# yezhen17/3DIoUMatch

Hardware: AMD Instinct MI355X
Metric: scenes/sec train-step (ScanNet 40k pts, 256 proposals) (higher is better)
Workload: dtype f32

## Files before the change

### 3dioumatch_amd/_lib.py

```python
import ctypes
import os

_HERE = os.path.dirname(os.path.abspath(__file__))
LIB_PATH = os.path.join(_HERE, "lib3dioumatch_hip%s.so" % os.environ.get("PN2_LIB_SUFFIX", ""))

_c_int, _c_float, _vp, _sz = ctypes.c_int, ctypes.c_float, ctypes.c_void_p, ctypes.c_size_t


class MlpOperand(ctypes.Structure):
    _fields_ = [("mode", _c_int), ("x", _vp), ("dz", _vp), ("scale", _vp), ("shift", _vp), ("mean", _vp),
                ("invstd", _vp), ("coef", _vp), ("argmax", _vp), ("ns", _c_int), ("groups", _c_int),
                ("lin_w", _vp)]


_op = ctypes.POINTER(MlpOperand)

_SIGNATURES = {
    "pn2_furthest_point_sampling": [_c_int, _c_int, _c_int, _vp, _vp, _vp, _vp],
    "pn2_furthest_point_sampling_ws": [_c_int, _c_int, _c_int, _vp, _vp, _vp, _sz, _vp],
    "pn2_fps_workspace_bytes": [_c_int, _c_int, _c_int],
    "pn2_gather_points": [_c_int, _c_int, _c_int, _c_int, _vp, _vp, _vp, _vp],
    "pn2_gather_points_grad": [_c_int, _c_int, _c_int, _c_int, _vp, _vp, _vp, _vp],
    "pn2_ball_query": [_c_int, _c_int, _c_int, _c_float, _c_int, _vp, _vp, _vp, _vp, _sz, _vp],
    "pn2_ball_query_workspace_bytes": [_c_int, _c_int, _c_int, _c_int],
# ... 40 lines not shown
    "mlp_bn_workspace_floats": [_c_int, _c_int, _c_int],
    "mlp_bn_train_stats": [_c_int, _c_int, _c_int, _vp, _vp, _vp, _c_float, _c_float, _vp, _vp, _vp,
                           _vp, _vp, _vp, _vp, _vp, _vp],
    "mlp_bn_eval_coeff": [_c_int, _vp, _vp, _c_float, _vp, _vp, _vp, _vp, _vp, _vp, _vp],
    "mlp_bn_relu_apply": [_c_int, _c_int, _c_int, _vp, _vp, _vp, _vp, _vp],
    "mlp_bn_relu_pool": [_c_int, _c_int, _c_int, _c_int, _vp, _vp, _vp, _vp, _vp, _vp, _vp],
    "mlp_bn_relu_backward": [_c_int, _c_int, _c_int, _c_int, _vp, _vp, _vp, _vp, _vp, _vp, _vp, _vp,
                             _vp, _vp, _vp, _vp, _vp, _vp],
    "mlp_bn_relu_pool_backward": [_c_int, _c_int, _c_int, _c_int, _c_int, _vp, _vp, _vp, _vp, _vp,
                                  _vp, _vp, _vp, _vp, _vp, _vp, _vp, _vp, _vp, _vp, _vp],
    "mlp_bn_relu_backward_stats": [_c_int, _c_int, _c_int, _c_int, _vp, _vp, _vp, _vp, _vp, _vp,
                                   _vp, _vp, _vp, _vp, _vp, _vp, _vp],
    "mlp_gemm_forward": [_c_int] * 4 + [_vp, _vp, _op, _vp, _vp, _vp],
    "mlp_gemm_forward_small": [_c_int] * 4 + [_vp, _c_int, _vp, _op, _vp, _vp, _vp],
    "mlp_gemm_forward_stats_parts": [_c_int, _c_int, _c_int, _c_int, _vp],
    "mlp_bn_finalize_pairs": [_c_int, _c_int, _c_int, _vp, _vp, _vp, _c_float, _c_float, _vp, _vp,
                              _vp, _vp, _vp, _vp, _vp, _vp],
    "mlp_bn_finalize_pairs_scratch_bytes": [_c_int],
    "mlp_gemm_dgrad": [_c_int] * 4 + [_vp, _op, _vp, _vp],
    "mlp_gemm_wgrad": [_c_int] * 4 + [_op, _op, _vp, _vp, _vp],
    "mlp_gemm_wgrad_workspace_floats": [_c_int, _c_int, _c_int, _c_int],
    "mlp_gemm_forward_stats_pool_supported": [_c_int, _c_int, _c_int, _c_int, _c_int],
    "mlp_gemm_forward_stats_pool": [_c_int] * 4 + [_vp, _op, _vp, _vp, _c_int, _vp, _vp, _vp],
    "mlp_pool_gram_supported": [_c_int] * 5,
    "mlp_pool_gram_parts": [_c_int] * 4,
    "mlp_pool_gram_workspace_floats": [_c_int] * 5,
    "mlp_pool_gram_backward": [_c_int] * 4 + [_vp, _op, _op] + [_vp] * 6,
    "mlp_eval_lin4_supported": [_c_int] * 6,
    "mlp_eval_lin4_pool": [_c_int, _c_int, _c_int, _vp, _vp, _vp, _vp, _vp, _vp, _vp, _vp],
    "mlp_eval_stored_supported": [_c_int] * 6,
    "mlp_eval_stored_tiles_per_wave": [_c_int] * 4,
    "mlp_eval_stored_image_bytes": [_c_int],
    "mlp_eval_stored_prepare": [_c_int, _vp, _vp, _vp, _vp],
    "mlp_eval_stored_pool": [_c_int, _c_int, _c_int, _c_int, _vp, _vp, _vp, _vp, _vp, _vp, _vp, _vp, _vp, _vp],
    "mlp_chain_lin4_parts": [_c_int, _c_int, _c_int, _c_int, _vp],
    "mlp_chain_lin4_image_bytes": [],
    "mlp_chain_lin4_prepare": [_vp, _vp, _vp, _vp, _vp, _vp, _vp],
    "mlp_chain_lin4_stats": [_c_int, _c_int, _c_int, _vp, _vp, _vp, _vp],
    "mlp_chain_lin4_forward": [_c_int, _c_int, _c_int, _vp, _vp, _vp, _vp, _vp, _vp, _vp, _vp, _vp, _vp],
    "mlp_chain_finalize": [_c_int, _c_int, _c_int, _vp, _vp, _vp, _c_float, _c_float, _vp, _vp, _vp, _vp, _vp,
                           _vp, _vp],
    "mlp_bn_pool_from_extrema": [_c_int, _c_int, _c_int, _vp, _vp, _vp, _vp, _vp, _vp, _vp],
    "mlp_wgrad_first4_workspace_bytes": [_c_int, _c_int],
    "mlp_wgrad_first4": [_c_int, _c_int, _vp, _vp, _vp, _vp, _vp, _vp, _vp, _vp, _vp, _vp, _vp, _vp],
    "mlp_wgrad_first4_from_gated": [_c_int] + [_vp] * 9,
    "mlp_first4_moments_doubles": [],
# ... 124 lines not shown
```

### 3dioumatch_amd/csrc/mlp_gemm.hip

```cpp
#include "common.h"
#include "mlp_operand.h"
#include <mutex>
#include <stdlib.h>

namespace {

constexpr int KC = 16;

template <int TM, int TN, int WM, int WN, int MODE, bool A_TRANS>
__global__ void __launch_bounds__(256)
gemm_nn_kernel(int m_total, int k_total, int r, const float *__restrict__ a, int lda, OperandB opb,
               float *__restrict__ c, size_t b_stride_in, size_t b_stride_out) {
  constexpr int MB = TM / WM / 32, NB = TN / WN / 32;
  constexpr int LDA = TM + 4;
  __shared__ float As[KC * LDA];
  __shared__ __attribute__((aligned(16))) float Bs[KC * TN];
  const int tid = threadIdx.x, lane = tid & 63, wave = tid >> 6;
  const int wm = wave / WN, wn = wave % WN;
  const int r0 = blockIdx.x * TN, m0 = blockIdx.y * TM, b = blockIdx.z;
  OperandB op = opb;
  const size_t in_off = (size_t)b * b_stride_in;

  f32x16 acc[MB][NB];
#pragma unroll
// ... 1249 lines not shown
    return launch_nn<OP_BNRELU>(b, m, k, r, w, ldw, op, y, in_stride, out_stride, stream, nullptr, ai);
  }
  const dim3 grid(pn2_ceil_div(r, 64), pn2_ceil_div(m, 64), b);
#define BIAS_FORM(MODE)                                                                                  \
  do {                                                                                                   \
    if (img)                                                                                             \
      hipLaunchKernelGGL((gemm_nn_small_bias_kernel<MODE, true>), grid, dim3(256), 0, stream, m, k, r, w, \
                         ldw, op, y, in_stride, out_stride, ai, bias);                                   \
    else                                                                                                 \
      hipLaunchKernelGGL((gemm_nn_small_bias_kernel<MODE, false>), grid, dim3(256), 0, stream, m, k, r,  \
                         w, ldw, op, y, in_stride, out_stride, ai, bias);                                \
  } while (0)
  if (x->mode == OP_DIRECT) BIAS_FORM(OP_DIRECT);
  else BIAS_FORM(OP_BNRELU);
#undef BIAS_FORM
  return pn2_launch_status();
}

MLP_API int mlp_gemm_forward_stats_pool_supported(int b, int m, int k, int r, int ns) {
  if (mlp_gemm_forward_stats_parts(b, m, k, r, nullptr) == 0) return 0;
  return (m == 128 || m == 256) && (ns == 16 || ns == 32 || ns == 64) && r % ns == 0 && k % 4 == 0;
}

MLP_API int mlp_gemm_forward_stats_pool(int b, int m, int k, int r, const float *w, const MlpOperand *x,
                                        float *y, float *pairs, int ns, const float *gamma, float *ext,
                                        void *stream_) {
  if (!mlp_gemm_forward_stats_pool_supported(b, m, k, r, ns)) return (int)hipErrorInvalidValue;
  OperandB op;
  const int rc = operand_from_abi(x, op_bit(OP_BNRELU), r, &op);
  if (rc) return rc;
  if (!pairs || !ext || !gamma || (reinterpret_cast<size_t>(w) & 15) != 0) return (int)hipErrorInvalidValue;
  hipStream_t stream = (hipStream_t)stream_;
  if (mlp_pool_fwd256_supported(b, m, k, r, ns, w, *x) && (reinterpret_cast<size_t>(y) & 15) == 0)
    return mlp_pool_fwd256_launch(b, r, ns, w, *x, gamma, y, pairs, ext, stream);
  const size_t in_stride = (size_t)k * r, out_stride = (size_t)m * r;
  const size_t plane = (size_t)b * m * (r / ns);
  const unsigned a_bytes = (unsigned)(4 * (size_t)m * k);
#define POOLED(TM, TN, WM, WN, NS)                                                                 \
  hipLaunchKernelGGL((gemm_nn2_kernel<TM, TN, WM, WN, OP_BNRELU, false, true, true, NS>),          \
                     dim3(r / TN, 1, b), dim3(256), 0, stream, m, k, r, w, k, a_bytes, op, y,     \
                     in_stride, out_stride, pairs, m, ext, plane, gamma)
  if (m == 256 && ns == 16) POOLED(256, 64, 4, 1, 16);
  else if (m == 256 && ns == 32) POOLED(256, 64, 4, 1, 32);
  else if (m == 256) POOLED(256, 64, 4, 1, 64);
  else if (ns == 16) POOLED(128, 128, 2, 2, 16);
  else if (ns == 32) POOLED(128, 128, 2, 2, 32);
  else POOLED(128, 128, 2, 2, 64);
#undef POOLED
  return pn2_launch_status();
}

MLP_API int mlp_gemm_dgrad(int b, int m, int k, int r, const float *w, const MlpOperand *dy,
                           float *dx, void *stream_) {
  if (b <= 0 || m <= 0 || k <= 0 || r <= 0) return 0;
  OperandB op;
  const int rc = operand_from_abi(dy, op_bit(OP_DIRECT) | op_bit(OP_DY) | op_bit(OP_POOLDY), r, &op);
  if (rc) return rc;
  const size_t in_stride = (size_t)m * r, out_stride = (size_t)k * r;
  hipStream_t stream = (hipStream_t)stream_;
  if (dy->mode == OP_DIRECT)
    return launch_nn<OP_DIRECT, true>(b, k, m, r, w, k, op, dx, in_stride, out_stride, stream);
  if (dy->mode == OP_DY)
    return launch_nn<OP_DY, true>(b, k, m, r, w, k, op, dx, in_stride, out_stride, stream);
  return launch_nn<OP_POOLDY, true>(b, k, m, r, w, k, op, dx, in_stride, out_stride, stream);
}

static bool wgrad_direct_ok(int b, int m, int k, int r, int pmode, int qmode);
static int wgrad_direct_r_per_slice(int b, int m, int k, int r);

MLP_API int mlp_gemm_backward_small_supported(int b, int m, int k, int r, int pmode, int qmode) {
  return b > 0 && m > 0 && k > 0 && (long long)b * r <= small_gemm_cols() &&
         wgrad_direct_ok(b, m, k, r, pmode, qmode);
// ... 147 lines not shown
```

### 3dioumatch_amd/csrc/mlp_operand.h

```cpp
#pragma once
#include "common.h"
#include "mlp_frag.h"
#include "../../include/mlp_hip.h"

namespace {

enum OperandMode { OP_DIRECT = 0, OP_BNRELU = 1, OP_DY = 2, OP_POOLDY = 3, OP_LIN4 = 4 };

struct OperandB {
  const float *x;
  const float *dz;
  const float *scale;
  const float *shift;
  const float *mean;
  const float *invstd;
  const float *coef;
  const int *argmax;
  int ns;
  int groups;
  const float *lin_w;
};

constexpr bool is_dy(int mode) { return mode == OP_DY || mode == OP_POOLDY; }

// ... 83 lines not shown
        if (MODE == OP_DY) {
          const float4 d = *reinterpret_cast<const float4 *>(op.dz + off + i);
          dz[i] = d.x; dz[i + 1] = d.y; dz[i + 2] = d.z; dz[i + 3] = d.w;
        }
      }
    }
  } else {
#pragma unroll
    for (int i = 0; i < N; ++i) {
      if (gr + i < limit) {
        x[i] = op.x[off + i];
        if (MODE == OP_DY) dz[i] = op.dz[off + i];
      }
    }
  }
}

}

int mlp_reduce_partials(int count, int parts, const float *part, float *out, hipStream_t stream);
int mlp_reduce_weight_partials(int count, int parts, const float *part, float *out, hipStream_t stream);
int mlp_pool_fwd256_supported(int b, int m, int k, int r, int ns, const float *w, const MlpOperand &x);
int mlp_pool_fwd256_launch(int b, int r, int ns, const float *w, const MlpOperand &x, const float *gamma,
                           float *y, float *pairs, float *ext, hipStream_t stream);
bool mlp_pool_gram256_supported(int b, int r, int ns);
int mlp_pool_gram256_parts(int b, int r);
size_t mlp_pool_gram256_workspace_floats(int b, int r, int ns);
int mlp_pool_gram256_launch(int b, int r, const float *w, const MlpOperand &dy, const MlpOperand &x,
                            const float *ymax, float *dq, float *dw, float *stats_part, float *workspace,
                            hipStream_t stream);
```

### 3dioumatch_amd/csrc/mlp_pool_fwd256.hip

```cpp
#include "common.h"
#include "mlp_operand.h"
#include <stdlib.h>
#include <type_traits>

namespace {

constexpr int kFM = 256, kFK = 128, kFTN = 32;
constexpr int kFRP = kFTN * 2;
constexpr int kFIMG = kFK * kFRP;
constexpr int kFBUF = 3 * kFIMG;
constexpr int kFTP = 32 * 144;

struct PoolFwdArgs {
  int r, chunks_per_cloud, total_tiles, groups;
  const float *w;
  const float *x;
  const float *sc, *sh;
  const float *gamma;
  float *pairs;
  float *ext;
  size_t ext_plane;
  float *y;
};

typedef float f_f32x2 __attribute__((ext_vector_type(2)));
typedef float f_f32x4 __attribute__((ext_vector_type(4)));

template <int NS, bool STORE>
__global__ void __launch_bounds__(512) pool_fwd256_kernel(const PoolFwdArgs a) {
  constexpr int K = kFK, TN = kFTN, RP = kFRP, IMG = kFIMG, BUF = kFBUF;
  constexpr int G = TN / NS;
  constexpr int QG = 16 / G;
  static_assert(NS == 16 || NS == 32, "nsample");
  extern __shared__ __attribute__((aligned(16))) char lds[];

  const int tid = threadIdx.x, lane = tid & 63;
  const int wave = __builtin_amdgcn_readfirstlane(tid >> 6);
  const int l31 = lane & 31, lhi = lane >> 5;
  const int seg_row = tid >> 3, seg_c = (tid & 7) * 4;
  const int ch = 32 * wave + l31;

  Split3 wsp[K / 16];
  {
    const float *wr = a.w + (size_t)ch * K + 8 * lhi;
#pragma unroll
    for (int s = 0; s < K / 16; ++s)
      wsp[s] = split3(*reinterpret_cast<const float4 *>(wr + 16 * s),
                      *reinterpret_cast<const float4 *>(wr + 16 * s + 4));
  }
  const bool neg = a.gamma[ch] < 0.f;
  const float sg = neg ? -1.f : 1.f;
  const f_f32x2 sgn = {sg, sg};
  const RowCoef rc0 = {a.sc[seg_row], a.sh[seg_row], 0.f, 0.f, 0.f};
  const RowCoef rc1 = {a.sc[seg_row + 64], a.sh[seg_row + 64], 0.f, 0.f, 0.f};

  const int blocks = a.total_tiles / 2;
  const int per = (blocks + (int)gridDim.x - 1) / (int)gridDim.x;
  const int k_lo = (int)blockIdx.x * per;
  const int k_hi = k_lo + per < blocks ? k_lo + per : blocks;
  const int c_lo = 4 * k_lo, c_hi = 4 * k_hi;
  if (c_lo >= c_hi) return;

  float4 qx0, qx1, qf0, qf1;
  auto fetch = [&](int c) {
    const int b = c / a.chunks_per_cloud;
    const int col0 = (c - b * a.chunks_per_cloud) * TN;
    const float *src = a.x + ((size_t)b * K + seg_row) * a.r + col0 + seg_c;
    qf0 = *reinterpret_cast<const float4 *>(src);
    qf1 = *reinterpret_cast<const float4 *>(src + (size_t)64 * a.r);
  };
  auto stage_slice = [&](char *base, int row, const float4 &x, const RowCoef &rc) {
    const float xv[4] = {x.x, x.y, x.z, x.w};
    float h[4], m[4], l[4];
#pragma unroll
    for (int e = 0; e < 4; ++e) split_terms(transform<OP_BNRELU>(xv[e], 0.f, rc), h[e], m[e], l[e]);
    store_terms4<RP>(base, IMG, row, seg_c, h, m, l);
  };
  auto stage = [&](char *base) {
    stage_slice(base, seg_row, qx0, rc0);
    stage_slice(base, seg_row + 64, qx1, rc1);
  };
  auto clampc = [&](int c) { return c < c_hi ? c : c_hi - 1; };

  const int tr_off = (8 * lhi + ((lane & 15) >> 2)) * RP + (16 * ((lane >> 4) & 1) + 4 * (lane & 3)) * 2;
  bf16x4 pf[2][3][2];
  auto frag = [&](const char *Q, int s, bf16x4 (&dst)[3][2]) {
#pragma unroll
    for (int t = 0; t < 3; ++t) {
      const char *p0 = Q + (size_t)t * IMG + (size_t)(16 * s) * RP + tr_off;
      dst[t][0] = lds_read_tr(p0);
      dst[t][1] = lds_read_tr(p0 + 4 * RP);
    }
  };
  auto operand = [&](const bf16x4 (&src)[3][2]) {
    Split3 sb;
    sb.hi = __builtin_shufflevector(src[0][0], src[0][1], 0, 1, 2, 3, 4, 5, 6, 7);
    sb.mid = __builtin_shufflevector(src[1][0], src[1][1], 0, 1, 2, 3, 4, 5, 6, 7);
    sb.lo = __builtin_shufflevector(src[2][0], src[2][1], 0, 1, 2, 3, 4, 5, 6, 7);
    return sb;
  };

  fetch(c_lo);
  qx0 = qf0; qx1 = qf1;
  stage(lds);
  fetch(clampc(c_lo + 1));
  qx0 = qf0; qx1 = qf1;
  fetch(clampc(c_lo + 2));
  __syncthreads();
  frag(lds, 0, pf[0]);

  float tsh = 0.f;
  f_f32x2 t1 = {0.f, 0.f}, t2 = {0.f, 0.f};
  unsigned held[4] = {0u, 0u, 0u, 0u};
  int cur = 0;

  float sv[4], shh[4], sm[4], sl[4];
  f_f32x2 pv[8];
  float best[G], mh = 0.f, qh = 0.f, mo = 0.f, qo = 0.f;
  float ob[G];
  int at[G], oa[G];
  char *Qn = lds;
  int ce = 0;
  bool real = false;
  f_f32x4 yrow[2];
  auto store_rows = [&](int k0) {
    if (real) {
      const int b = ce / a.chunks_per_cloud;
      float *dst = a.y + ((size_t)b * kFM + 32 * wave + (lane >> 3)) * a.r + (ce - b * a.chunks_per_cloud) * TN + 4 * (lane & 7);
#pragma unroll
      for (int k2 = 0; k2 < 2; ++k2)
        __builtin_nontemporal_store(yrow[k2], reinterpret_cast<f_f32x4 *>(dst + (size_t)(8 * (k0 + k2)) * a.r));
    }
  };
  auto piece = [&](auto nt) {
    constexpr int n = decltype(nt)::value;
    if constexpr (n == 0 || n == 4) {
      const float4 &x = n == 0 ? qx0 : qx1;
      const RowCoef &rc = n == 0 ? rc0 : rc1;
      const float xv[4] = {x.x, x.y, x.z, x.w};
#pragma unroll
      for (int e = 0; e < 4; ++e) sv[e] = transform<OP_BNRELU>(xv[e], 0.f, rc);
    } else if constexpr (n == 1 || n == 5) {
#pragma unroll
      for (int e = 0; e < 4; ++e) split_top(sv[e], shh[e], sv[e]);
    } else if constexpr (n == 2 || n == 6) {
#pragma unroll
      for (int e = 0; e < 4; ++e) split_top(sv[e], sm[e], sl[e]);
    } else if constexpr (n == 3 || n == 7) {
      store_terms4<RP>(Qn, IMG, seg_row + (n == 7 ? 64 : 0), seg_c, shh, sm, sl);
    } else if constexpr (n == 8) {
      qx0 = qf0; qx1 = qf1;
      fetch(clampc(ce + 4));
    } else if constexpr (n == 9 || n == 10 || n == 11) {
      if (n == 9 && (ce & 1) == 0) { tsh = pv[0].x; t1 = f_f32x2{0.f, 0.f}; t2 = t1; }
      if constexpr (STORE) {
        char *tp = lds + 3 * BUF + wave * kFTP;
        if constexpr (n == 9) {
#pragma unroll
          for (int j = 0; j < 4; ++j)
            *reinterpret_cast<f_f32x4 *>(tp + l31 * 144 + 32 * j + 16 * lhi) =
                f_f32x4{pv[2 * j].x, pv[2 * j].y, pv[2 * j + 1].x, pv[2 * j + 1].y};
        } else if constexpr (n == 10) {
#pragma unroll
          for (int k2 = 0; k2 < 2; ++k2) yrow[k2] = *reinterpret_cast<const f_f32x4 *>(tp + (8 * k2 + (lane >> 3)) * 144 + (lane & 7) * 16);
        } else {
          store_rows(0);
#pragma unroll
          for (int k2 = 0; k2 < 2; ++k2) yrow[k2] = *reinterpret_cast<const f_f32x4 *>(tp + (8 * (k2 + 2) + (lane >> 3)) * 144 + (lane & 7) * 16);
        }
      }
      const f_f32x2 sh2 = {tsh, tsh};
#pragma unroll
      for (int j = 3 * (n - 9); j < (n == 11 ? 8 : 3 * (n - 8)); ++j) {
        const f_f32x2 d = pv[j] - sh2;
        t1 += d;
// ... 34 lines not shown
#pragma unroll
      for (int gq = 0; gq < G; ++gq) {
        float bb = best[gq];
        int aa = at[gq];
        if (ob[gq] > bb || (ob[gq] == bb && oa[gq] < aa)) { bb = ob[gq]; aa = oa[gq]; }
        if (aa == 64) aa = 0;
        const float out = bb * sg;
        held[0] = held[1]; held[1] = held[2]; held[2] = held[3];
        held[3] = lhi == 0 ? __builtin_bit_cast(unsigned, out) : (unsigned)aa;
      }
    } else if constexpr (n == 19) {
      if (ce & 1) {
        const float s1 = t1.x + t1.y, s2 = t2.x + t2.y;
        mh = tsh + s1 * (1.0f / 32.0f);
        qh = fmaxf(s2 - s1 * s1 * (1.0f / 32.0f), 0.f);
        mo = __shfl_xor(mh, 32, kWave);
        qo = __shfl_xor(qh, 32, kWave);
      }
    } else if constexpr (n == 20) {
      if ((ce & 1) && real && lhi == 0) {
        const float dlt = mo - mh;
        const float mean = 0.5f * (mh + mo);
        const float m2w = (qh + qo) + 16.0f * dlt * dlt;
        *reinterpret_cast<float2 *>(a.pairs + ((size_t)(ce >> 1) * kFM + ch) * 2) = make_float2(mean, m2w);
      }
    } else if constexpr (n == 21) {
      if ((ce & (4 / G - 1)) == 4 / G - 1 && real) {
        const int b = ce / a.chunks_per_cloud;
        const int g_last = ((ce - b * a.chunks_per_cloud) * TN) / NS + G - 1;
        const size_t o = ((size_t)b * kFM + ch) * a.groups + g_last - 3 + (lhi ? a.ext_plane : 0);
        *reinterpret_cast<uint4 *>(reinterpret_cast<unsigned *>(a.ext) + o) = make_uint4(held[0], held[1], held[2], held[3]);
      }
    }
  };
#define PF_PIECE(N) do { piece(std::integral_constant<int, (N)>{}); __builtin_amdgcn_sched_barrier(0); } while (0)

#pragma unroll
  for (int j = 0; j < 8; ++j) pv[j] = f_f32x2{0.f, 0.f};
  for (int c = c_lo; c < c_hi; ++c) {
    const int nxt = cur == 2 ? 0 : cur + 1;
    const char *Qc = lds + (size_t)cur * BUF;
    Qn = lds + (size_t)nxt * BUF;
    ce = c - 1;
    real = c > c_lo;
    f32x16 acc, acc1;
#pragma unroll
    for (int q = 0; q < 16; ++q) { acc[q] = 0.f; acc1[q] = 0.f; }
#pragma unroll
    for (int s = 0; s < K / 16; ++s) {
      const int ring = s & 1;
      if (s + 1 < K / 16) frag(Qc, s + 1, pf[ring ^ 1]);
      else frag(Qn, 0, pf[ring ^ 1]);
      __builtin_amdgcn_sched_barrier(0);
      const Split3 x = operand(pf[ring]);
      const Split3 &w = wsp[s];
#define PF_MM(AT, BT)                                                                                \
  acc = __builtin_amdgcn_mfma_f32_32x32x16_bf16(x.AT, w.BT, acc, 0, 0, 0);
#define PF_MM1(AT, BT)                                                                               \
  acc1 = __builtin_amdgcn_mfma_f32_32x32x16_bf16(x.AT, w.BT, acc1, 0, 0, 0);
#define PF_CASE(N) case N: PF_PIECE(N); break
      PF_MM(lo, hi) PF_MM1(hi, lo)
      switch (3 * s) {
        PF_CASE(0); PF_CASE(3); PF_CASE(6); PF_CASE(9); PF_CASE(12); PF_CASE(15); PF_CASE(18); PF_CASE(21);
      }
      PF_MM(mid, mid) PF_MM1(mid, hi)
      switch (3 * s + 1) {
        PF_CASE(1); PF_CASE(4); PF_CASE(7); PF_CASE(10); PF_CASE(13); PF_CASE(16); PF_CASE(19);
      }
      PF_MM(hi, mid) PF_MM1(hi, hi)
      switch (3 * s + 2) {
        PF_CASE(2); PF_CASE(5); PF_CASE(8); PF_CASE(11); PF_CASE(14); PF_CASE(20);
      }
#undef PF_CASE
#undef PF_MM
#undef PF_MM1
      if (s == 3) __syncthreads();
    }
    cur = nxt;
#pragma unroll
    for (int j = 0; j < 8; ++j) pv[j] = f_f32x2{acc[2 * j], acc[2 * j + 1]} + f_f32x2{acc1[2 * j], acc1[2 * j + 1]};
  }
  ce = c_hi - 1;
  real = true;
  PF_PIECE(9); PF_PIECE(10); PF_PIECE(11); PF_PIECE(12); PF_PIECE(13); PF_PIECE(14); PF_PIECE(15);
  PF_PIECE(16); PF_PIECE(18); PF_PIECE(19); PF_PIECE(20); PF_PIECE(21);
#undef PF_PIECE
}

}

int mlp_pool_fwd256_supported(int b, int m, int k, int r, int ns, const float *w, const MlpOperand &x) {
  const char *env = getenv("MLP_POOL_FWD256");
  const bool off = env && atoi(env) == 0;
  if (off || b <= 0 || m != kFM || k != kFK || r <= 0 || r % 256 != 0) return 0;
  if ((ns != 16 && ns != 32) || r % ns != 0) return 0;
  return ((reinterpret_cast<size_t>(w) | reinterpret_cast<size_t>(x.x)) & 15) == 0 ? 1 : 0;
}

int mlp_pool_fwd256_launch(int b, int r, int ns, const float *w, const MlpOperand &x, const float *gamma,
                           float *y, float *pairs, float *ext, hipStream_t stream) {
  if (!w || !x.x || !x.scale || !x.shift || !gamma || !pairs || !ext || (ns != 16 && ns != 32) || b <= 0 || r <= 0 ||
      r % 256 != 0)
    return (int)hipErrorInvalidValue;
  PoolFwdArgs a = {};
  a.r = r; a.chunks_per_cloud = r / kFTN; a.total_tiles = b * (r / 64); a.groups = r / ns;
  a.w = w; a.x = x.x; a.sc = x.scale; a.sh = x.shift; a.gamma = gamma; a.pairs = pairs; a.ext = ext; a.y = y;
  a.ext_plane = (size_t)b * kFM * (size_t)(r / ns);
  int grid = pn2_cu_count();
  if (grid > a.total_tiles / 2) grid = a.total_tiles / 2;
  const size_t kLds = 3 * (size_t)kFBUF + (y != nullptr ? 8 * (size_t)kFTP : 0);
  constexpr size_t kLdsMax = 3 * (size_t)kFBUF + 8 * (size_t)kFTP;
  for (const void *kern : {reinterpret_cast<const void *>(pool_fwd256_kernel<16, false>),
                           reinterpret_cast<const void *>(pool_fwd256_kernel<32, false>),
                           reinterpret_cast<const void *>(pool_fwd256_kernel<16, true>),
                           reinterpret_cast<const void *>(pool_fwd256_kernel<32, true>)})
    pn2_allow_dynamic_lds(kern, kLdsMax);
  if (y != nullptr) {
    if (ns == 16) hipLaunchKernelGGL((pool_fwd256_kernel<16, true>), dim3(grid), dim3(512), kLds, stream, a);
    else hipLaunchKernelGGL((pool_fwd256_kernel<32, true>), dim3(grid), dim3(512), kLds, stream, a);
  } else {
    if (ns == 16) hipLaunchKernelGGL((pool_fwd256_kernel<16, false>), dim3(grid), dim3(512), kLds, stream, a);
    else hipLaunchKernelGGL((pool_fwd256_kernel<32, false>), dim3(grid), dim3(512), kLds, stream, a);
  }
  return pn2_launch_status();
}
```

### 3dioumatch_amd/dropin/pointnet2/_mlp_ext.py

```python
import contextlib
import ctypes
import os

import torch

from pointnet2._ext import _L, _lib, _stream

SMALL_BWD_DY_COLS = 4096


def _f32c(t, name):
    if t.dtype != torch.float32 or not t.is_contiguous() or not t.is_cuda:
        raise RuntimeError("%s must be a contiguous float32 GPU tensor" % name)


def _ws(y, b, c, r):
    n = int(_lib.mlp_bn_workspace_floats(b, c, r))
    return torch.empty(max(n, 1), dtype=torch.float32, device=y.device)


def new_tickets(channels, device):
    return torch.zeros(max(int(channels), 1), dtype=torch.int32, device=device)


def tickets_of(module, channels, device):
    t = module.__dict__.get("_pn2_tickets")
    if t is None or t.device != device or t.numel() < channels:
        t = new_tickets(channels, device)
        module.__dict__["_pn2_tickets"] = t
    return t


def _tk(tickets, c, ref):
    if tickets is None:
        return new_tickets(c, ref.device)
    if tickets.dtype != torch.int32 or tickets.device != ref.device or tickets.numel() < c or \
            not tickets.is_contiguous():
        raise RuntimeError("tickets must be a contiguous int32 tensor of >= %d zeros on %s" % (c, ref.device))
    return tickets


def bn_coefficients(y, gamma, beta, running_mean, running_var, momentum, eps, training, tickets=None):
    _f32c(y, "y")
    b, c = y.shape[0], y.shape[1]
    r = y.numel() // (b * c)
    out = torch.empty((4, c), dtype=torch.float32, device=y.device)
    mean, invstd, scale, shift = out[0], out[1], out[2], out[3]
    with torch.cuda.device(y.device):
        if training:
            ws = _ws(y, b, c, r)
            rm = running_mean.data_ptr() if running_mean is not None else None
            rv = running_var.data_ptr() if running_var is not None else None
            _L.check(_lib.mlp_bn_train_stats(b, c, r, y.data_ptr(), gamma.data_ptr(),
                                             beta.data_ptr(), float(eps), float(momentum), rm, rv,
                                             mean.data_ptr(), invstd.data_ptr(), scale.data_ptr(),
                                             shift.data_ptr(), ws.data_ptr(),
                                             _tk(tickets, c, y).data_ptr(), _stream(y)),
                     "mlp_bn_train_stats")
        else:
            _L.check(_lib.mlp_bn_eval_coeff(c, gamma.data_ptr(), beta.data_ptr(), float(eps),
                                            running_mean.data_ptr(), running_var.data_ptr(),
                                            mean.data_ptr(), invstd.data_ptr(), scale.data_ptr(),
# ... 220 lines not shown
    y = torch.empty((b, m) + tuple(x.shape[2:]), dtype=torch.float32, device=x.device)
    image = _image_of(w, b, r)
    op = _input_operand(x, coeff)
    with torch.cuda.device(x.device):
        _L.check(_lib.mlp_gemm_forward(b, m, k, r, w.data_ptr(), image[0] if image else None,
                                       ctypes.byref(op), y.data_ptr(), None, _stream(x)),
                 "mlp_gemm_forward")
    return y


def _finalize_pairs(c, parts, n_part, pairs, gamma, beta, running_mean, running_var, momentum, eps):
    out = torch.empty((4, c), dtype=torch.float32, device=pairs.device)
    scratch = torch.empty(int(_lib.mlp_bn_finalize_pairs_scratch_bytes(c)), dtype=torch.uint8,
                          device=pairs.device)
    _L.check(_lib.mlp_bn_finalize_pairs(c, parts, n_part, pairs.data_ptr(), gamma.data_ptr(),
                                        beta.data_ptr(), float(eps), float(momentum),
                                        _ptr(running_mean), _ptr(running_var), out[0].data_ptr(),
                                        out[1].data_ptr(), out[2].data_ptr(), out[3].data_ptr(),
                                        scratch.data_ptr(), _stream(pairs)), "mlp_bn_finalize_pairs")
    return out[0], out[1], out[2], out[3]


def gemm_forward_bn(w, x, coeff, gamma, beta, running_mean, running_var, momentum, eps, pool=False,
                    tickets=None, store=True):
    _f32c(x, "x"); _f32c(w, "w")
    b, k = x.shape[0], x.shape[1]
    r = x.numel() // (b * k)
    m = w.shape[0]
    cols = ctypes.c_int(0)
    parts = int(_lib.mlp_gemm_forward_stats_parts(b, m, k, r, ctypes.byref(cols)))
    if parts <= 0:
        y = gemm_forward(w, x, coeff)
        return (y,) + tuple(bn_coefficients(y, gamma, beta, running_mean, running_var, momentum,
                                            eps, True, tickets)) + ((None,) if pool else ())
    ns = x.shape[3] if (pool and x.dim() == 4) else 0
    pooled = bool(ns) and coeff is not None and w.data_ptr() % 16 == 0 and \
        bool(_lib.mlp_gemm_forward_stats_pool_supported(b, m, k, r, ns))
    ext = torch.empty((2, b, m, r // ns), dtype=torch.float32, device=x.device) if pooled else None
    if not store and not pooled:
        raise RuntimeError("gemm_forward_bn(store=False): the pooled epilogue does not cover this layer")
    y = torch.empty((b, m) + tuple(x.shape[2:]), dtype=torch.float32, device=x.device) if store else None
    pairs = torch.empty((parts, m, 2), dtype=torch.float32, device=x.device)
    op = _input_operand(x, coeff)
    with torch.cuda.device(x.device):
        if pooled:
            _L.check(_lib.mlp_gemm_forward_stats_pool(b, m, k, r, w.data_ptr(), ctypes.byref(op), _ptr(y),
                                                      pairs.data_ptr(), ns, gamma.data_ptr(),
                                                      ext.data_ptr(), _stream(x)),
                     "mlp_gemm_forward_stats_pool")
        else:
            _L.check(_lib.mlp_gemm_forward(b, m, k, r, w.data_ptr(), None, ctypes.byref(op),
                                           y.data_ptr(), pairs.data_ptr(), _stream(x)),
                     "mlp_gemm_forward(pairs)")
        bn = _finalize_pairs(m, parts, cols.value, pairs, gamma, beta, running_mean, running_var,
                             momentum, eps)
    return (y,) + bn + ((ext,) if pool else ())


def forward_pool_supported(w, x, coeff):
    shape = x if isinstance(x, tuple) else tuple(x.shape)
    if len(shape) != 4 or coeff is None or w.data_ptr() % 16 != 0:
        return False
    b, k, m, ns = shape
    return bool(_lib.mlp_gemm_forward_stats_pool_supported(b, w.shape[0], k, m * ns, ns))


def pool_from_extrema(ext, scale, shift):
    _, b, c, m = ext.shape
# ... 489 lines not shown
```

### 3dioumatch_amd/dropin/pointnet2/pytorch_utils.py

```python
import contextlib
import os

import torch
import torch.nn as nn
from torch.autograd import Function


class _BNBase(nn.Sequential):

    def __init__(self, in_size, batch_norm=None, name=""):
        super().__init__()
        layer = batch_norm(in_size)
        nn.init.constant_(layer.weight, 1.0)
        nn.init.constant_(layer.bias, 0)
        self.add_module(name + "bn", layer)


class BatchNorm1d(_BNBase):
    def __init__(self, in_size, *, name=""):
        super().__init__(in_size, batch_norm=nn.BatchNorm1d, name=name)


class BatchNorm2d(_BNBase):
    def __init__(self, in_size, name=""):
# ... 142 lines not shown
        raise RuntimeError("the pre-gather form needs src_ext (B, 3+C, n+m) and two layers or more")
    first = "plain"
    if isinstance(pre, Pregathered):
        first = "pregathered"
    elif isinstance(pre, Interpolated):
        first = "interpolated"
    elif training and n >= 3 and x.dim() == 4 and not input_grad and K.lin4_supported(ws[0], ws[1], x):
        chained = pool and n == 3 and K.chain_lin4_supported(ws[0], ws[1], ws[2], x, x.shape[3])
        first = "chained" if chained else "virtual"
    if not pool:
        return first, "apply"
    b, m, ns = pre.extent if pre is not None else (x.shape[0], x.shape[2], x.shape[3])
    y_in = (b, ws[-1].shape[1], m, ns)
    if first == "chained":
        return first, "gram" if K.pool_gram_supported(ws[2], y_in, ns) else "extrema"
    if not (training and n >= 2 and K.forward_pool_supported(ws[-1], y_in, True)):
        return first, "bn_relu_pool"
    return first, "gram" if K.pool_gram_supported(ws[-1], y_in, ns) else "extrema"


class _FusedMLPChain(Function):

    @staticmethod
    def forward(ctx, x, pool, training, momenta, epss, pre, tickets, *params):
        from pointnet2 import _mlp_ext as K
        n = len(params) // 5
        x = x.contiguous()
        ws = [w.reshape(w.shape[0], -1) for w in params[0::5]]
        bns = [tuple(params[5 * i + 1:5 * i + 5]) + (momenta[i], epss[i]) for i in range(n)]
        first, last = chain_forms(ws, x, pre, pool, training, ctx.needs_input_grad[0])
        store = any(ctx.needs_input_grad)
        ys, coefs = [], []
        moments, ext = None, None
        if first in ("virtual", "chained"):
            moments = K.first4_moments(x)
            ys.append(None)
            coefs.append(K.first4_bn(moments, x.numel() // 4, ws[0], *bns[0]))
        if first == "chained":
            y1, c1, y2, c2, ext = K.chain_lin4_forward(x, ws[0], coefs[0][2:], (ws[1],) + bns[1],
                                                       (ws[2],) + bns[2], store=store, store_last=last != "gram")
            ys += [y1, y2]
            coefs += [c1, c2]
        elif first == "virtual":
            y, *c = K.gemm_forward_bn_lin4(ws[1], x, ws[0], coefs[0][2:], *bns[1])
            ys.append(y)
            coefs.append(tuple(c))
        elif first == "pregathered" and training:
            y, *c = pre.forward(ws[0], x, bns[0])
            ys.append(y)
            coefs.append(tuple(c))
        elif pre is not None:
            ys.append(pre.forward(ws[0], x))
            coefs.append(K.bn_coefficients(ys[0], *bns[0], training, tickets))
        for i in range(len(ys), n):
            cur, coeff = (x, None) if i == 0 else (ys[i - 1], coefs[i - 1][2:])
            if i == n - 1 and last in ("extrema", "gram"):
                y, *c, ext = K.gemm_forward_bn(ws[i], cur, coeff, *bns[i], pool=True, tickets=tickets,
                                               store=store and last == "extrema")
            elif training:
                y, *c = K.gemm_forward_bn(ws[i], cur, coeff, *bns[i], tickets=tickets)
            else:
                y = K.gemm_forward(ws[i], cur, coeff)
                c = K.bn_coefficients(y, *bns[i], False, tickets)
            ys.append(y)
            coefs.append(tuple(c))
        scale, shift = coefs[-1][2:]
        argmax = ymax = None
        if last == "apply":
            out = K.bn_relu_apply(ys[-1], scale, shift)
        elif last == "bn_relu_pool":
            out, argmax, ymax = K.bn_relu_pool(ys[-1], scale, shift)
        else:
            out, argmax, ymax = K.pool_from_extrema(ext, scale, shift)
        ctx.save_for_backward(x, moments, argmax, ymax, *ys, *[t for c in coefs for t in c], *params)
        ctx.n_layers, ctx.training, ctx.tickets, ctx.pre = n, training, tickets, pre
        ctx.first, ctx.last = first, last
        return out

    @staticmethod
    def backward(ctx, dout):
        from pointnet2 import _mlp_ext as K
# ... 39 lines not shown
            if i == 0 and first == "pregathered":
                dw, dz = ctx.pre.backward(ws[0], x, grad["fly"], need_dx)
                grads[0] = dw.view_as(params[0])
                break
            lin_w = ws[0] if (i == 1 and virtual) else None
            src = x if (i == 0 or lin_w is not None) else ys[i - 1]
            src_coeff = None if i == 0 else coefs[i - 1][2:]
            src_stats = None if i == 0 else coefs[i - 1][:2] + (params[5 * i - 4], training)
            fused = None if "dy" in grad else K.gemm_backward_fused(
                ws[i], src, src_coeff, xstats=src_stats, need_dx=i > 0 or need_dx, lin_w=lin_w, **grad)
            if fused is not None:
                dsrc, dw, below = fused
            elif lin_w is not None:
                raise RuntimeError("the virtual first layer needs the fused backward kernel of the second")
            elif i == 0 and not need_dx:
                dsrc, below = None, None
                dw = K.wgrad_first4(ws[0], x, grad["fly"]) if "fly" in grad else None
                if dw is None:
                    dw = K.gemm_wgrad(ws[0].shape[0], ws[0].shape[1], x, None, **grad)
            else:
                (dw, dsrc), below = K.both(ws[i], src, src_coeff, **grad), None
            grads[5 * i] = dw.view_as(params[5 * i])
            dz = dsrc
        return (dz if need_dx else None, None, None, None, None, None, None, *grads)


_deferred_counters = None
_deferred_axpy = None
zero_grads_as_none = False


@contextlib.contextmanager
def deferred_bn_counters():
    global _deferred_counters, _deferred_axpy
    previous, _deferred_counters = _deferred_counters, []
    previous_axpy, _deferred_axpy = _deferred_axpy, []
    try:
        yield
    finally:
        pending, _deferred_counters = _deferred_counters, previous
        axpy, _deferred_axpy = _deferred_axpy, previous_axpy
        if pending:
            torch._foreach_add_(pending, 1)
        by_alpha = {}
        for t, other, alpha in axpy:
            by_alpha.setdefault(float(alpha), ([], []))
            by_alpha[float(alpha)][0].append(t)
# ... 45 lines not shown
            return False
        conv, bn_wrap, act = kids["conv"], kids["bn"], kids["activation"]
        bns = list(bn_wrap.children())
        return (isinstance(conv, nn.Conv2d) and conv.kernel_size == (1, 1) and conv.bias is None
                and conv.stride == (1, 1) and conv.padding == (0, 0) and len(bns) == 1
                and isinstance(bns[0], nn.BatchNorm2d) and bns[0].affine
                and bns[0].track_running_stats and bns[0].momentum is not None
                and isinstance(act, nn.ReLU))

    def _use_fused(self, x):
        return (x.is_cuda and x.dtype == torch.float32 and x.dim() == 4 and len(self) > 0
                and all(self._fusable(layer) for layer in self))

    def _run(self, x, pool, pre=None):
        from pointnet2 import _mlp_ext as K
        if _eval_plans is not None and pool:
            plan = _eval_plans.get(id(self))
            if plan is not None and plan.mlp is self:
                out = plan.run(x, pre)
                if out is not None:
                    return out
        layers = list(self)
        tickets = K.tickets_of(self, max(layer.conv.out_channels for layer in layers), x.device)
        bns = [next(layer.bn.children()) for layer in layers]
        training = bns[0].training
        if all(bn.training == training for bn in bns):
            params = []
            for layer, bn in zip(layers, bns):
                if training:
                    bump_batches_tracked(bn.num_batches_tracked)
                params += [layer.conv.weight, bn.weight, bn.bias, bn.running_mean,
                           bn.running_var]
            return _FusedMLPChain.apply(x, pool, training, [bn.momentum for bn in bns],
                                        [bn.eps for bn in bns], pre, tickets, *params)
        for i, layer in enumerate(layers):
            bn = next(layer.bn.children())
            y = layer.conv(x)
            training = bn.training
            if training:
                bump_batches_tracked(bn.num_batches_tracked)
            op = _BNReLUMaxPool if (pool and i == len(layers) - 1) else _BNReLU
            x = op.apply(y, bn.weight, bn.bias, bn.running_mean, bn.running_var, bn.momentum,
                         bn.eps, training, tickets)
        return x

    def forward(self, x):
        if self._use_fused(x):
            return self._run(x, pool=False)
        return super().forward(x)

    def pregather_ok(self, xyz, new_xyz, features, m, ns):
        if features is None or len(self) < 2:
            return False
        if not (features.is_cuda and features.dtype == torch.float32
                and all(self._fusable(layer) for layer in self)):
            return False
        bns = [next(layer.bn.children()) for layer in self]
# ... 178 lines not shown
```

### include/mlp_hip.h

```cpp
#ifndef MLP_HIP_H
#define MLP_HIP_H

#include <stddef.h>

#ifdef __cplusplus
extern "C" {
#endif

size_t mlp_bn_workspace_floats(int b, int c, int r);


int mlp_bn_train_stats(int b, int c, int r, const float *y, const float *gamma, const float *beta,
                       float eps, float momentum, float *running_mean, float *running_var,
                       float *mean, float *invstd, float *scale, float *shift, float *workspace,
                       int *tickets, void *stream);

int mlp_bn_eval_coeff(int c, const float *gamma, const float *beta, float eps,
                      const float *running_mean, const float *running_var, float *mean,
                      float *invstd, float *scale, float *shift, void *stream);

int mlp_bn_relu_apply(int b, int c, int r, const float *y, const float *scale, const float *shift,
                      float *z, void *stream);

int mlp_bn_relu_pool(int b, int c, int m, int ns, const float *y, const float *scale,
// ... 34 lines not shown

int mlp_gemm_forward(int b, int m, int k, int r, const float *w, const void *img,
                     const MlpOperand *x, float *y, float *pairs, void *stream);
int mlp_gemm_forward_small(int b, int m, int k, int r, const float *w, int ldw, const void *img,
                           const MlpOperand *x, const float *bias, float *y, void *stream);

int mlp_gemm_forward_stats_parts(int b, int m, int k, int r, int *cols_per_part);
int mlp_bn_finalize_pairs(int c, int parts, int n_part, const float *pairs, const float *gamma,
                          const float *beta, float eps, float momentum, float *running_mean,
                          float *running_var, float *mean, float *invstd, float *scale,
                          float *shift, void *scratch, void *stream);
size_t mlp_bn_finalize_pairs_scratch_bytes(int c);

int mlp_gemm_dgrad(int b, int m, int k, int r, const float *w, const MlpOperand *dy, float *dx,
                   void *stream);

int mlp_gemm_wgrad(int b, int m, int k, int r, const MlpOperand *dy, const MlpOperand *x,
                   float *dw, float *workspace, void *stream);

int mlp_gemm_forward_stats_pool_supported(int b, int m, int k, int r, int ns);
int mlp_gemm_forward_stats_pool(int b, int m, int k, int r, const float *w, const MlpOperand *x,
                                float *y, float *pairs, int ns, const float *gamma, float *ext,
                                void *stream);
int mlp_chain_lin4_parts(int b, int r, int m3, int ns, int *cols_per_part);
size_t mlp_chain_lin4_image_bytes(void);
int mlp_chain_lin4_prepare(const float *w1, const float *sc1, const float *sh1, const float *w2,
                           const float *w3, void *img, void *stream);
int mlp_chain_lin4_stats(int b, int r, int ns, const float *x4, const void *img, float *pairs2,
                         void *stream);
int mlp_chain_lin4_forward(int b, int r, int ns, const float *x4, const void *img, const float *sc2,
                           const float *sh2, const float *gamma3, float *y2, float *y3, float *pairs3,
                           float *ext, void *stream);
int mlp_chain_finalize(int c, int parts, int n_part, const float *pairs, const float *gamma,
                       const float *beta, float eps, float momentum, float *running_mean,
                       float *running_var, float *mean, float *invstd, float *scale, float *shift,
                       void *stream);
int mlp_pool_gram_supported(int b, int m, int k, int r, int ns);
int mlp_pool_gram_parts(int b, int m, int k, int r);
size_t mlp_pool_gram_workspace_floats(int b, int m, int k, int r, int ns);
int mlp_pool_gram_backward(int b, int m, int k, int r, const float *w, const MlpOperand *dy,
                           const MlpOperand *x, const float *ymax, float *dq, float *dw,
                           float *stats_part, float *workspace, void *stream);
int mlp_bn_pool_from_extrema(int b, int c, int groups, const float *ext, const float *scale,
                             const float *shift, float *pooled, int *argmax, float *ymax,
                             void *stream);

// ... 63 lines not shown
```

Measured before the change: 1420.

## Schedule pooled fwd256 GEMM tiles via an atomic work queue

Replaces the static contiguous per-block tile partition in the fused pooled forward kernel with dynamic work stealing. Each workgroup draws runs of tiles from a device atomic counter, prefetching the next ticket through LDS slots, and the counter wraps so it self-resets for reuse. The aim is to balance load across CUs and reduce tail imbalance. The cost is atomic traffic, extra control logic in the pipelined loop, and a per-module queue tensor. An env var can cap the grid size.

```diff
diff --git a/3dioumatch_amd/_lib.py b/3dioumatch_amd/_lib.py
--- a/3dioumatch_amd/_lib.py
+++ b/3dioumatch_amd/_lib.py
@@ -86,6 +86,7 @@
     "mlp_gemm_wgrad_workspace_floats": [_c_int, _c_int, _c_int, _c_int],
     "mlp_gemm_forward_stats_pool_supported": [_c_int, _c_int, _c_int, _c_int, _c_int],
     "mlp_gemm_forward_stats_pool": [_c_int] * 4 + [_vp, _op, _vp, _vp, _c_int, _vp, _vp, _vp],
+    "mlp_gemm_forward_stats_pool_queued": [_c_int] * 4 + [_vp, _op, _vp, _vp, _c_int, _vp, _vp, _vp, _vp],
     "mlp_pool_gram_supported": [_c_int] * 5,
     "mlp_pool_gram_parts": [_c_int] * 4,
     "mlp_pool_gram_workspace_floats": [_c_int] * 5,
diff --git a/3dioumatch_amd/csrc/mlp_gemm.hip b/3dioumatch_amd/csrc/mlp_gemm.hip
--- a/3dioumatch_amd/csrc/mlp_gemm.hip
+++ b/3dioumatch_amd/csrc/mlp_gemm.hip
@@ -1295,9 +1295,9 @@
   return (m == 128 || m == 256) && (ns == 16 || ns == 32 || ns == 64) && r % ns == 0 && k % 4 == 0;
 }
 
-MLP_API int mlp_gemm_forward_stats_pool(int b, int m, int k, int r, const float *w, const MlpOperand *x,
-                                        float *y, float *pairs, int ns, const float *gamma, float *ext,
-                                        void *stream_) {
+static int forward_stats_pool(int b, int m, int k, int r, const float *w, const MlpOperand *x, float *y,
+                              float *pairs, int ns, const float *gamma, float *ext, unsigned *queue,
+                              void *stream_) {
   if (!mlp_gemm_forward_stats_pool_supported(b, m, k, r, ns)) return (int)hipErrorInvalidValue;
   OperandB op;
   const int rc = operand_from_abi(x, op_bit(OP_BNRELU), r, &op);
@@ -1305,7 +1305,7 @@
   if (!pairs || !ext || !gamma || (reinterpret_cast<size_t>(w) & 15) != 0) return (int)hipErrorInvalidValue;
   hipStream_t stream = (hipStream_t)stream_;
   if (mlp_pool_fwd256_supported(b, m, k, r, ns, w, *x) && (reinterpret_cast<size_t>(y) & 15) == 0)
-    return mlp_pool_fwd256_launch(b, r, ns, w, *x, gamma, y, pairs, ext, stream);
+    return mlp_pool_fwd256_launch(b, r, ns, w, *x, gamma, y, pairs, ext, queue, stream);
   const size_t in_stride = (size_t)k * r, out_stride = (size_t)m * r;
   const size_t plane = (size_t)b * m * (r / ns);
   const unsigned a_bytes = (unsigned)(4 * (size_t)m * k);
@@ -1321,6 +1321,20 @@
   else POOLED(128, 128, 2, 2, 64);
 #undef POOLED
   return pn2_launch_status();
+}
+
+MLP_API int mlp_gemm_forward_stats_pool(int b, int m, int k, int r, const float *w, const MlpOperand *x,
+                                        float *y, float *pairs, int ns, const float *gamma, float *ext,
+                                        void *stream_) {
+  return forward_stats_pool(b, m, k, r, w, x, y, pairs, ns, gamma, ext, nullptr, stream_);
+}
+
+MLP_API int mlp_gemm_forward_stats_pool_queued(int b, int m, int k, int r, const float *w,
+                                               const MlpOperand *x, float *y, float *pairs, int ns,
+                                               const float *gamma, float *ext, unsigned *queue,
+                                               void *stream_) {
+  if ((reinterpret_cast<size_t>(queue) & 3) != 0) return (int)hipErrorInvalidValue;
+  return forward_stats_pool(b, m, k, r, w, x, y, pairs, ns, gamma, ext, queue, stream_);
 }
 
 MLP_API int mlp_gemm_dgrad(int b, int m, int k, int r, const float *w, const MlpOperand *dy,
diff --git a/3dioumatch_amd/csrc/mlp_operand.h b/3dioumatch_amd/csrc/mlp_operand.h
--- a/3dioumatch_amd/csrc/mlp_operand.h
+++ b/3dioumatch_amd/csrc/mlp_operand.h
@@ -129,7 +129,7 @@
 int mlp_reduce_weight_partials(int count, int parts, const float *part, float *out, hipStream_t stream);
 int mlp_pool_fwd256_supported(int b, int m, int k, int r, int ns, const float *w, const MlpOperand &x);
 int mlp_pool_fwd256_launch(int b, int r, int ns, const float *w, const MlpOperand &x, const float *gamma,
-                           float *y, float *pairs, float *ext, hipStream_t stream);
+                           float *y, float *pairs, float *ext, unsigned *queue, hipStream_t stream);
 bool mlp_pool_gram256_supported(int b, int r, int ns);
 int mlp_pool_gram256_parts(int b, int r);
 size_t mlp_pool_gram256_workspace_floats(int b, int r, int ns);
diff --git a/3dioumatch_amd/csrc/mlp_pool_fwd256.hip b/3dioumatch_amd/csrc/mlp_pool_fwd256.hip
--- a/3dioumatch_amd/csrc/mlp_pool_fwd256.hip
+++ b/3dioumatch_amd/csrc/mlp_pool_fwd256.hip
@@ -21,6 +21,7 @@
   float *ext;
   size_t ext_plane;
   float *y;
+  unsigned *queue;
 };
 
 typedef float f_f32x2 __attribute__((ext_vector_type(2)));
@@ -40,6 +41,18 @@
   const int seg_row = tid >> 3, seg_c = (tid & 7) * 4;
   const int ch = 32 * wave + l31;
 
+  constexpr int RC = NS == 32 ? 4 : 2;
+  __shared__ unsigned q_slot[2];
+  const bool queued = a.queue != nullptr;
+  const unsigned runs = (unsigned)(2 * a.total_tiles / RC);
+  unsigned tk = 0u;
+  auto draw = [&]() { tk = __builtin_amdgcn_atomic_inc32(a.queue, runs + gridDim.x - 1u, __ATOMIC_RELAXED, "agent"); };
+  auto post = [&](int slot) {
+    if (tid == 0) q_slot[slot] = tk;
+    tk = 0u;
+  };
+  if (queued && tid == 0) draw();
+
   Split3 wsp[K / 16];
   {
     const float *wr = a.w + (size_t)ch * K + 8 * lhi;
@@ -48,18 +61,55 @@
       wsp[s] = split3(*reinterpret_cast<const float4 *>(wr + 16 * s),
                       *reinterpret_cast<const float4 *>(wr + 16 * s + 4));
   }
+  const size_t ext_lane = (size_t)ch * a.groups + (lhi ? a.ext_plane : 0);
+  const size_t y_lane = (size_t)(lane >> 3) * a.r + 4 * (lane & 7);
   const bool neg = a.gamma[ch] < 0.f;
   const float sg = neg ? -1.f : 1.f;
   const f_f32x2 sgn = {sg, sg};
   const RowCoef rc0 = {a.sc[seg_row], a.sh[seg_row], 0.f, 0.f, 0.f};
   const RowCoef rc1 = {a.sc[seg_row + 64], a.sh[seg_row + 64], 0.f, 0.f, 0.f};
 
-  const int blocks = a.total_tiles / 2;
-  const int per = (blocks + (int)gridDim.x - 1) / (int)gridDim.x;
-  const int k_lo = (int)blockIdx.x * per;
-  const int k_hi = k_lo + per < blocks ? k_lo + per : blocks;
-  const int c_lo = 4 * k_lo, c_hi = 4 * k_hi;
-  if (c_lo >= c_hi) return;
+  int g_c = 0, g_left = 0, g_id = 0, g_adv = 0, ahead = 0, post_slot = -1;
+  bool g_end = false;
+  if (queued) {
+    post(0);
+    __syncthreads();
+  } else {
+    const int blocks = a.total_tiles / 2;
+    const int per = (blocks + (int)gridDim.x - 1) / (int)gridDim.x;
+    const int k_lo = (int)blockIdx.x * per;
+    const int k_hi = k_lo + per < blocks ? k_lo + per : blocks;
+    g_c = 4 * k_lo;
+    g_left = 4 * (k_hi - k_lo);
+    g_end = true;
+  }
+  auto take = [&]() {
+    if (g_left > 0) { g_id = g_c; ++g_c; --g_left; ++ahead; }
+    return g_id;
+  };
+  auto next = [&]() {
+    if (g_left <= 0 && !g_end) {
+      const unsigned t = __builtin_amdgcn_readfirstlane(q_slot[g_adv & 1]);
+      if (t < runs) {
+        g_c = RC * (int)t;
+        g_left = RC;
+        post_slot = (g_adv + 1) & 1;
+      } else {
+        g_end = true;
+      }
+      ++g_adv;
+    }
+    return take();
+  };
+  auto draw_due = [&]() {
+    if (post_slot >= 0 && tid == 0) draw();
+  };
+  auto post_due = [&]() {
+    if (post_slot >= 0) { post(post_slot); post_slot = -1; }
+  };
+  int w0 = next(), w1, w2, w3;
+  if (ahead == 0) return;
+  draw_due();
 
   float4 qx0, qx1, qf0, qf1;
   auto fetch = [&](int c) {
@@ -80,7 +130,6 @@
     stage_slice(base, seg_row, qx0, rc0);
     stage_slice(base, seg_row + 64, qx1, rc1);
   };
-  auto clampc = [&](int c) { return c < c_hi ? c : c_hi - 1; };
 
   const int tr_off = (8 * lhi + ((lane & 15) >> 2)) * RP + (16 * ((lane >> 4) & 1) + 4 * (lane & 3)) * 2;
   bf16x4 pf[2][3][2];
@@ -100,14 +149,19 @@
     return sb;
   };
 
-  fetch(c_lo);
+  fetch(w0);
   qx0 = qf0; qx1 = qf1;
   stage(lds);
-  fetch(clampc(c_lo + 1));
+  w1 = take();
+  fetch(w1);
   qx0 = qf0; qx1 = qf1;
-  fetch(clampc(c_lo + 2));
+  post_due();
   __syncthreads();
+  w2 = next();
+  draw_due();
+  fetch(w2);
   frag(lds, 0, pf[0]);
+  post_due();
 
   float tsh = 0.f;
   f_f32x2 t1 = {0.f, 0.f}, t2 = {0.f, 0.f};
@@ -120,13 +174,13 @@
   float ob[G];
   int at[G], oa[G];
   char *Qn = lds;
-  int ce = 0;
+  int ce = -1;
   bool real = false;
   f_f32x4 yrow[2];
   auto store_rows = [&](int k0) {
     if (real) {
       const int b = ce / a.chunks_per_cloud;
-      float *dst = a.y + ((size_t)b * kFM + 32 * wave + (lane >> 3)) * a.r + (ce - b * a.chunks_per_cloud) * TN + 4 * (lane & 7);
+      float *dst = a.y + ((size_t)b * kFM + 32 * wave) * a.r + (ce - b * a.chunks_per_cloud) * TN + y_lane;
 #pragma unroll
       for (int k2 = 0; k2 < 2; ++k2)
         __builtin_nontemporal_store(yrow[k2], reinterpret_cast<f_f32x4 *>(dst + (size_t)(8 * (k0 + k2)) * a.r));
@@ -150,7 +204,8 @@
       store_terms4<RP>(Qn, IMG, seg_row + (n == 7 ? 64 : 0), seg_c, shh, sm, sl);
     } else if constexpr (n == 8) {
       qx0 = qf0; qx1 = qf1;
-      fetch(clampc(ce + 4));
+      fetch(w3);
+      draw_due();
     } else if constexpr (n == 9 || n == 10 || n == 11) {
       if (n == 9 && (ce & 1) == 0) { tsh = pv[0].x; t1 = f_f32x2{0.f, 0.f}; t2 = t1; }
       if constexpr (STORE) {
@@ -231,14 +286,15 @@
         const float dlt = mo - mh;
         const float mean = 0.5f * (mh + mo);
         const float m2w = (qh + qo) + 16.0f * dlt * dlt;
-        *reinterpret_cast<float2 *>(a.pairs + ((size_t)(ce >> 1) * kFM + ch) * 2) = make_float2(mean, m2w);
+        float *tile_pairs = a.pairs + (size_t)(ce >> 1) * (kFM * 2);
+        *reinterpret_cast<float2 *>(tile_pairs + 2 * ch) = make_float2(mean, m2w);
       }
     } else if constexpr (n == 21) {
       if ((ce & (4 / G - 1)) == 4 / G - 1 && real) {
         const int b = ce / a.chunks_per_cloud;
         const int g_last = ((ce - b * a.chunks_per_cloud) * TN) / NS + G - 1;
-        const size_t o = ((size_t)b * kFM + ch) * a.groups + g_last - 3 + (lhi ? a.ext_plane : 0);
-        *reinterpret_cast<uint4 *>(reinterpret_cast<unsigned *>(a.ext) + o) = make_uint4(held[0], held[1], held[2], held[3]);
+        const size_t o = (size_t)b * kFM * a.groups + (g_last - 3);
+        *reinterpret_cast<uint4 *>(reinterpret_cast<unsigned *>(a.ext) + (o + ext_lane)) = make_uint4(held[0], held[1], held[2], held[3]);
       }
     }
   };
@@ -246,12 +302,11 @@
 
 #pragma unroll
   for (int j = 0; j < 8; ++j) pv[j] = f_f32x2{0.f, 0.f};
-  for (int c = c_lo; c < c_hi; ++c) {
+  while (ahead > 0) {
     const int nxt = cur == 2 ? 0 : cur + 1;
     const char *Qc = lds + (size_t)cur * BUF;
     Qn = lds + (size_t)nxt * BUF;
-    ce = c - 1;
-    real = c > c_lo;
+    w3 = next();
     f32x16 acc, acc1;
 #pragma unroll
     for (int q = 0; q < 16; ++q) { acc[q] = 0.f; acc1[q] = 0.f; }
@@ -285,12 +340,14 @@
 #undef PF_MM1
       if (s == 3) __syncthreads();
     }
+    post_due();
     cur = nxt;
+    ce = w0; w0 = w1; w1 = w2; w2 = w3;
+    real = true;
+    --ahead;
 #pragma unroll
     for (int j = 0; j < 8; ++j) pv[j] = f_f32x2{acc[2 * j], acc[2 * j + 1]} + f_f32x2{acc1[2 * j], acc1[2 * j + 1]};
   }
-  ce = c_hi - 1;
-  real = true;
   PF_PIECE(9); PF_PIECE(10); PF_PIECE(11); PF_PIECE(12); PF_PIECE(13); PF_PIECE(14); PF_PIECE(15);
   PF_PIECE(16); PF_PIECE(18); PF_PIECE(19); PF_PIECE(20); PF_PIECE(21);
 #undef PF_PIECE
@@ -307,7 +364,7 @@
 }
 
 int mlp_pool_fwd256_launch(int b, int r, int ns, const float *w, const MlpOperand &x, const float *gamma,
-                           float *y, float *pairs, float *ext, hipStream_t stream) {
+                           float *y, float *pairs, float *ext, unsigned *queue, hipStream_t stream) {
   if (!w || !x.x || !x.scale || !x.shift || !gamma || !pairs || !ext || (ns != 16 && ns != 32) || b <= 0 || r <= 0 ||
       r % 256 != 0)
     return (int)hipErrorInvalidValue;
@@ -315,8 +372,16 @@
   a.r = r; a.chunks_per_cloud = r / kFTN; a.total_tiles = b * (r / 64); a.groups = r / ns;
   a.w = w; a.x = x.x; a.sc = x.scale; a.sh = x.shift; a.gamma = gamma; a.pairs = pairs; a.ext = ext; a.y = y;
   a.ext_plane = (size_t)b * kFM * (size_t)(r / ns);
+  a.queue = queue;
   int grid = pn2_cu_count();
-  if (grid > a.total_tiles / 2) grid = a.total_tiles / 2;
+  if (queue) {
+    const int runs = 2 * a.total_tiles / (ns == 32 ? 4 : 2);
+    const char *cap = getenv("MLP_POOL_FWD256_WGS");
+    if (cap && atoi(cap) > 0 && atoi(cap) < grid) grid = atoi(cap);
+    if (grid > runs) grid = runs;
+  } else if (grid > a.total_tiles / 2) {
+    grid = a.total_tiles / 2;
+  }
   const size_t kLds = 3 * (size_t)kFBUF + (y != nullptr ? 8 * (size_t)kFTP : 0);
   constexpr size_t kLdsMax = 3 * (size_t)kFBUF + 8 * (size_t)kFTP;
   for (const void *kern : {reinterpret_cast<const void *>(pool_fwd256_kernel<16, false>),
diff --git a/3dioumatch_amd/dropin/pointnet2/_mlp_ext.py b/3dioumatch_amd/dropin/pointnet2/_mlp_ext.py
--- a/3dioumatch_amd/dropin/pointnet2/_mlp_ext.py
+++ b/3dioumatch_amd/dropin/pointnet2/_mlp_ext.py
@@ -38,6 +38,25 @@
             not tickets.is_contiguous():
         raise RuntimeError("tickets must be a contiguous int32 tensor of >= %d zeros on %s" % (c, ref.device))
     return tickets
+
+
+def new_queue(device):
+    return torch.zeros(1, dtype=torch.int32, device=device)
+
+
+def queue_of(module, device):
+    q = module.__dict__.get("_pn2_queue")
+    if q is None or q.device != device:
+        q = new_queue(device)
+        module.__dict__["_pn2_queue"] = q
+    return q
+
+
+def _qw(queue, ref):
+    if queue.dtype != torch.int32 or queue.device != ref.device or queue.numel() < 1 or \
+            not queue.is_contiguous():
+        raise RuntimeError("queue must be a contiguous int32 tensor of one zero on %s" % (ref.device,))
+    return queue
 
 
 def bn_coefficients(y, gamma, beta, running_mean, running_var, momentum, eps, training, tickets=None):
@@ -304,8 +323,10 @@
 
 
 def gemm_forward_bn(w, x, coeff, gamma, beta, running_mean, running_var, momentum, eps, pool=False,
-                    tickets=None, store=True):
+                    tickets=None, store=True, queue=None):
     _f32c(x, "x"); _f32c(w, "w")
+    if queue is not None:
+        _qw(queue, x)
     b, k = x.shape[0], x.shape[1]
     r = x.numel() // (b * k)
     m = w.shape[0]
@@ -325,7 +346,13 @@
     pairs = torch.empty((parts, m, 2), dtype=torch.float32, device=x.device)
     op = _input_operand(x, coeff)
     with torch.cuda.device(x.device):
-        if pooled:
+        if pooled and queue is not None:
+            _L.check(_lib.mlp_gemm_forward_stats_pool_queued(b, m, k, r, w.data_ptr(), ctypes.byref(op),
+                                                             _ptr(y), pairs.data_ptr(), ns,
+                                                             gamma.data_ptr(), ext.data_ptr(),
+                                                             queue.data_ptr(), _stream(x)),
+                     "mlp_gemm_forward_stats_pool_queued")
+        elif pooled:
             _L.check(_lib.mlp_gemm_forward_stats_pool(b, m, k, r, w.data_ptr(), ctypes.byref(op), _ptr(y),
                                                       pairs.data_ptr(), ns, gamma.data_ptr(),
                                                       ext.data_ptr(), _stream(x)),
diff --git a/3dioumatch_amd/dropin/pointnet2/pytorch_utils.py b/3dioumatch_amd/dropin/pointnet2/pytorch_utils.py
--- a/3dioumatch_amd/dropin/pointnet2/pytorch_utils.py
+++ b/3dioumatch_amd/dropin/pointnet2/pytorch_utils.py
@@ -188,7 +188,7 @@
 class _FusedMLPChain(Function):
 
     @staticmethod
-    def forward(ctx, x, pool, training, momenta, epss, pre, tickets, *params):
+    def forward(ctx, x, pool, training, momenta, epss, pre, tickets, queue, *params):
         from pointnet2 import _mlp_ext as K
         n = len(params) // 5
         x = x.contiguous()
@@ -222,7 +222,7 @@
             cur, coeff = (x, None) if i == 0 else (ys[i - 1], coefs[i - 1][2:])
             if i == n - 1 and last in ("extrema", "gram"):
                 y, *c, ext = K.gemm_forward_bn(ws[i], cur, coeff, *bns[i], pool=True, tickets=tickets,
-                                               store=store and last == "extrema")
+                                               store=store and last == "extrema", queue=queue)
             elif training:
                 y, *c = K.gemm_forward_bn(ws[i], cur, coeff, *bns[i], tickets=tickets)
             else:
@@ -308,7 +308,7 @@
                 (dw, dsrc), below = K.both(ws[i], src, src_coeff, **grad), None
             grads[5 * i] = dw.view_as(params[5 * i])
             dz = dsrc
-        return (dz if need_dx else None, None, None, None, None, None, None, *grads)
+        return (dz if need_dx else None, None, None, None, None, None, None, None, *grads)
 
 
 _deferred_counters = None
@@ -400,6 +400,7 @@
                     return out
         layers = list(self)
         tickets = K.tickets_of(self, max(layer.conv.out_channels for layer in layers), x.device)
+        queue = K.queue_of(self, x.device) if pool else None
         bns = [next(layer.bn.children()) for layer in layers]
         training = bns[0].training
         if all(bn.training == training for bn in bns):
@@ -410,7 +411,7 @@
                 params += [layer.conv.weight, bn.weight, bn.bias, bn.running_mean,
                            bn.running_var]
             return _FusedMLPChain.apply(x, pool, training, [bn.momentum for bn in bns],
-                                        [bn.eps for bn in bns], pre, tickets, *params)
+                                        [bn.eps for bn in bns], pre, tickets, queue, *params)
         for i, layer in enumerate(layers):
             bn = next(layer.bn.children())
             y = layer.conv(x)
diff --git a/include/mlp_hip.h b/include/mlp_hip.h
--- a/include/mlp_hip.h
+++ b/include/mlp_hip.h
@@ -80,6 +80,9 @@
 int mlp_gemm_forward_stats_pool(int b, int m, int k, int r, const float *w, const MlpOperand *x,
                                 float *y, float *pairs, int ns, const float *gamma, float *ext,
                                 void *stream);
+int mlp_gemm_forward_stats_pool_queued(int b, int m, int k, int r, const float *w, const MlpOperand *x,
+                                       float *y, float *pairs, int ns, const float *gamma, float *ext,
+                                       unsigned *queue, void *stream);
 int mlp_chain_lin4_parts(int b, int r, int m3, int ns, int *cols_per_part);
 size_t mlp_chain_lin4_image_bytes(void);
 int mlp_chain_lin4_prepare(const float *w1, const float *sc1, const float *sh1, const float *w2,
```

Result: no change. 1430, median of 6 (+0.7%).
